# AliBahri94/GM3D

Hardware: AMD Instinct MI355X
Metric: point-clouds/sec pretrain step (N=1024,G=64) (higher is better)
Workload: dtype bf16

## Files before the change

gm3d_amd/csrc/attention.hip:

```cpp
#include "mfma.hpp"

namespace gm3d {

constexpr int HD = 64;
constexpr int VLD = 72;

__device__ __forceinline__ int permk(int s, int j, int hh) { return 16 * s + 8 * (j >> 2) + 4 * hh + (j & 3); }

__device__ __forceinline__ bf16x8 ld8(const bf16_t* p) { return *reinterpret_cast<const bf16x8*>(p); }
__device__ __forceinline__ bf16x8 ld8_perm(const bf16_t* row, int k0, int s, int hh) {
    const bf16x4 a = *reinterpret_cast<const bf16x4*>(row + k0 + 16 * s + 4 * hh);
    const bf16x4 b = *reinterpret_cast<const bf16x4*>(row + k0 + 16 * s + 8 + 4 * hh);
    bf16x8 v;
#pragma unroll
    for (int j = 0; j < 4; ++j) { v[j] = a[j]; v[4 + j] = b[j]; }
    return v;
}
__device__ __forceinline__ bf16x8 ld8_col_perm(const bf16_t* M, int ld, int k0, int s, int hh, int col) {
    bf16x8 v;
#pragma unroll
    for (int j = 0; j < 8; ++j) v[j] = M[(size_t)(k0 + permk(s, j, hh)) * ld + col];
    return v;
}

#define MFMA_F32(a, b, c) __builtin_amdgcn_mfma_f32_32x32x2f32(a, b, c, 0, 0, 0)

__device__ __forceinline__ void stage_bf16(bf16_t* dst , const bf16_t* src, size_t row_stride, int T, int rows) {
    for (int c = threadIdx.x; c < rows * 8; c += blockDim.x) {
        const int row = c >> 3, col = (c & 7) * 8;
        *reinterpret_cast<bf16x8*>(dst + row * VLD + col) = row < T ? ld8(src + (size_t)row * row_stride + col) : zero8();
    }
}
__device__ __forceinline__ int rot(int r, int c) { return r * 64 + ((c + r) & 63); }
__device__ __forceinline__ void stage_f32(float* dst , const float* src, size_t row_stride, int T, int rows) {
    for (int c = threadIdx.x; c < rows * 64; c += blockDim.x) {
        const int row = c >> 6, col = c & 63;
        dst[rot(row, col)] = row < T ? src[(size_t)row * row_stride + col] : 0.f;
    }
}

__device__ __forceinline__ int img_off(int row, int ch) {
    const int f = swz(row);
    return row * 128 + ((ch ^ f) << 4);
}
__device__ __forceinline__ bf16x8 img_row(const unsigned char* img, int row, int ch) {
    return *reinterpret_cast<const bf16x8*>(img + img_off(row, ch));
}
__device__ __forceinline__ bf16x4 img_tr(const unsigned char* img, int row0, int colblk, int lane) {
    const int l16 = lane & 15, q = l16 >> 2, p = l16 & 3;
    const int col = colblk + 4 * p;
    const int addr = img_off(row0 + q, col >> 3) + ((col >> 2) & 1) * 8;
    return __builtin_amdgcn_ds_read_tr16_b64_v4bf16((lds_bf16x4*)(img + addr));
}
__device__ __forceinline__ bf16x8 img_tr8(const unsigned char* img, int k0, int s, int hh, int colblk, int lane) {
    const bf16x4 lo = img_tr(img, k0 + 16 * s + 4 * hh, colblk, lane);
    const bf16x4 hi = img_tr(img, k0 + 16 * s + 8 + 4 * hh, colblk, lane);
    bf16x8 v;
#pragma unroll
    for (int j = 0; j < 4; ++j) { v[j] = lo[j]; v[4 + j] = hi[j]; }
    return v;
}
__device__ __forceinline__ void store_tile_t(unsigned char* img, int row0, const f32x16& x0, const f32x16& x1, int lane, bf16_t* g,
                                             size_t row_stride, int T) {
    const int r = lane & 31, hh = lane >> 5;
#pragma unroll
    for (int dt = 0; dt < 2; ++dt)
#pragma unroll
        for (int g4 = 0; g4 < 4; ++g4) {
            const f32x16& x = dt ? x1 : x0;
            bf16x4 pk;
#pragma unroll
            for (int e = 0; e < 4; ++e) pk[e] = (bf16_t)x[4 * g4 + e];
            *reinterpret_cast<bf16x4*>(img + img_off(row0 + r, 4 * dt + g4) + 8 * hh) = pk;
        }
    __builtin_amdgcn_fence(__ATOMIC_RELEASE, "wavefront");
    __builtin_amdgcn_wave_barrier();
    __builtin_amdgcn_fence(__ATOMIC_ACQUIRE, "wavefront");
#pragma unroll
    for (int i = 0; i < 4; ++i) {
        const int row = (lane >> 3) + 8 * i, ch = lane & 7;
        if (row0 + row < T)
            *reinterpret_cast<uint4*>(g + (size_t)(row0 + row) * row_stride + ch * 8) =
                *reinterpret_cast<const uint4*>(img + img_off(row0 + row, ch));
    }
}

template <int NT>
__device__ __forceinline__ void attn_core_bf16(const unsigned char* Qi, const unsigned char* Ki, const unsigned char* Vi,
                                               unsigned char* Oi, int w, int lane, int T, float scale, bf16_t* outp, size_t os,
                                               float* lsep) {
    const int r = lane & 31, hh = lane >> 5;
    f32x16 st[NT];
#pragma unroll
    for (int t = 0; t < NT; ++t) st[t] = zero16();
    const int qrow = 32 * w + r;
#pragma unroll
    for (int s = 0; s < 4; ++s) {
        const bf16x8 bq = img_row(Qi, qrow, 2 * s + hh);
#pragma unroll
        for (int t = 0; t < NT; ++t) st[t] = mfma_bf16(img_row(Ki, 32 * t + r, 2 * s + hh), bq, st[t]);
    }
    float m = -INFINITY;
#pragma unroll
    for (int t = 0; t < NT; ++t)
#pragma unroll
        for (int g = 0; g < 16; ++g) {
            const int key = 32 * t + crow(g, hh);
            st[t][g] = key < T ? st[t][g] * scale : -INFINITY;
            m = fmaxf(m, st[t][g]);
        }
    m = fmaxf(m, __shfl_xor(m, 32));
    float sum = 0.f;
#pragma unroll
    for (int t = 0; t < NT; ++t)
#pragma unroll
        for (int g = 0; g < 16; ++g) {
            st[t][g] = __expf(st[t][g] - m);
            sum += st[t][g];
        }
    sum += __shfl_xor(sum, 32);
    const float inv = 1.0f / sum;

    f32x16 o0 = zero16(), o1 = zero16();
    const int cb = 16 * ((lane >> 4) & 1);
#pragma unroll
    for (int t = 0; t < NT; ++t)
#pragma unroll
        for (int s = 0; s < 2; ++s) {
            const bf16x8 p = cvt8(st[t], s, inv);
            o0 = mfma_bf16(img_tr8(Vi, 32 * t, s, hh, cb, lane), p, o0);
            o1 = mfma_bf16(img_tr8(Vi, 32 * t, s, hh, 32 + cb, lane), p, o1);
        }
    store_tile_t(Oi, 32 * w, o0, o1, lane, outp, os, T);
    if (lsep && hh == 0 && qrow < T) lsep[qrow] = m + logf(sum);
}

template <int NT>
__global__ __launch_bounds__(64 * NT) void attn_fwd_bf16_kernel(const bf16_t* __restrict__ qkv, bf16_t* __restrict__ out,
                                                                float* __restrict__ lse, int T, int H, float scale) {
    extern __shared__ __attribute__((aligned(16))) unsigned char smem[];
    constexpr int ROWS = 32 * NT, IMG = ROWS * 128;
    unsigned char* Qi = smem;
    unsigned char* Ki = Qi + IMG;
    unsigned char* Vi = Ki + IMG;
    const int b = blockIdx.x / H, h = blockIdx.x % H;
    const int tid = threadIdx.x, lane = tid & 63, w = __builtin_amdgcn_readfirstlane(tid >> 6);
    const int r = lane & 31, hh = lane >> 5;
    const size_t rs = (size_t)3 * H * HD, os = (size_t)H * HD;
    const bf16_t* Qg = qkv + (size_t)b * T * rs + (size_t)h * HD;
    {
        uint4 v[12];
#pragma unroll
        for (int i = 0; i < 12; ++i) {
            const int c = tid + i * 64 * NT;
            const int tile = c / (ROWS * 8), rc = c - tile * (ROWS * 8), row = rc >> 3, ch = rc & 7;
            const int rr = row < T ? row : T - 1;
            v[i] = *reinterpret_cast<const uint4*>(Qg + (size_t)rr * rs + (size_t)tile * os + ch * 8);
        }
#pragma unroll
        for (int i = 0; i < 12; ++i) {
            const int c = tid + i * 64 * NT;
            const int tile = c / (ROWS * 8), rc = c - tile * (ROWS * 8), row = rc >> 3, ch = rc & 7;
            *reinterpret_cast<uint4*>(smem + tile * IMG + img_off(row, ch)) = row < T ? v[i] : make_uint4(0, 0, 0, 0);
        }
    }
    __syncthreads();

    attn_core_bf16<NT>(Qi, Ki, Vi, Qi, w, lane, T, scale, out + (size_t)b * T * os + (size_t)h * HD, os,
                       lse ? lse + ((size_t)b * H + h) * T : nullptr);
}

constexpr int QA_C = 384, QA_KT = QA_C / 64, QA_STAGE = (64 + 192) * 128;

template <int LOOK, bool WRITE_QKV>
__global__ __launch_bounds__(256) void attn_qkv_fwd_bf16_kernel(const bf16_t* __restrict__ hin, const bf16_t* __restrict__ wqkv,
                                                                bf16_t* __restrict__ out, float* __restrict__ lse,
                                                                bf16_t* __restrict__ qkv_out, int T, int H, float scale, int total) {
    extern __shared__ __attribute__((aligned(16))) unsigned char smem[];
    constexpr int NBUF = LOOK + 1;
    const int tid = threadIdx.x, lane = tid & 63, w = __builtin_amdgcn_readfirstlane(tid >> 6);
    const int r = lane & 31, hh = lane >> 5;
    const int logical = xcd_tile(blockIdx.x, gridDim.x);
    if (logical >= total) return;
    const int b = logical / H, h = logical - b * H;
    const unsigned lds0 = lds_addr(smem);

    const int prow = lane >> 3, pslot = lane & 7;
    const bf16_t* src[8];
#pragma unroll
    for (int i = 0; i < 8; ++i) {
        const int p = w + 4 * i;
        if (p < 8) {
            const int row = 8 * p + prow;
            const int t = row < T ? row : T - 1;
            const int f = (((row >> 1) & 1) << 2) | (((row >> 2) & 1) << 1) | ((row >> 3) & 1);
            src[i] = hin + ((size_t)b * T + t) * QA_C + ((pslot ^ f) << 3);
        } else {
            const int row = 8 * (p - 8) + prow;
            const int f = (((row >> 1) & 1) << 2) | (((row >> 2) & 1) << 1) | ((row >> 3) & 1);
            src[i] = wqkv + ((size_t)(row >> 6) * H * HD + (size_t)h * HD + (row & 63)) * QA_C + ((pslot ^ f) << 3);
        }
    }
#define GM3D_QA_STAGE(ST)                                                                        \
    {                                                                                            \
        const unsigned base = lds0 + ((ST) % NBUF) * QA_STAGE;                                   \
        _Pragma("unroll") for (int i = 0; i < 8; ++i) glds16(src[i] + (ST) * 64, base + 1024 * (w + 4 * i)); \
    }
    f32x16 acc[3];
#pragma unroll
    for (int j = 0; j < 3; ++j) acc[j] = zero16();
    const int wm = (w >> 1) * 32, wn = (w & 1) * 96;
#pragma unroll
    for (int s = 0; s < LOOK; ++s) GM3D_QA_STAGE(s)
#define GM3D_QA_ITER(KT_)                                                                                                   \
    {                                                                                                                       \
        asm volatile("s_waitcnt vmcnt(%0) lgkmcnt(0)" ::"n"(8 * ((QA_KT - 1 - (KT_)) < (LOOK - 1) ? (QA_KT - 1 - (KT_)) : (LOOK - 1))) : "memory"); \
        __builtin_amdgcn_s_barrier();                                                                                       \
        if ((KT_) + LOOK < QA_KT) GM3D_QA_STAGE((KT_) + LOOK)                                                               \
        const unsigned char* as = smem + ((KT_) % NBUF) * QA_STAGE;                                                         \
        const unsigned char* ws = as + 64 * 128;                                                                            \
        _Pragma("unroll") for (int s = 0; s < 4; ++s) {                                                                     \
            const bf16x8 fa = img_row(as, wm + r, 2 * s + hh);                                                              \
            _Pragma("unroll") for (int j = 0; j < 3; ++j) acc[j] = mfma_bf16(img_row(ws, wn + 32 * j + r, 2 * s + hh), fa, acc[j]); \
        }                                                                                                                   \
    }
    GM3D_QA_ITER(0) GM3D_QA_ITER(1) GM3D_QA_ITER(2) GM3D_QA_ITER(3) GM3D_QA_ITER(4) GM3D_QA_ITER(5)
#undef GM3D_QA_ITER
#undef GM3D_QA_STAGE
    static_assert((QA_KT - 1) % NBUF != 0, "the last stage must not sit in buffer 0");
    unsigned char* Qi = smem;
    unsigned char* Ki = smem + 8192;
    unsigned char* Vi = smem + 16384;
    unsigned char* Oi = smem + 24576;
    {
        const int token = wm + r;
#pragma unroll
        for (int j = 0; j < 3; ++j) {
            const int col = wn + 32 * j;
            unsigned char* img = smem + (col >> 6) * 8192;
            const int cbase = (col & 63) >> 3;
#pragma unroll
            for (int q = 0; q < 4; ++q) {
                bf16x4 pk;
#pragma unroll
                for (int e = 0; e < 4; ++e) pk[e] = token < T ? (bf16_t)acc[j][4 * q + e] : (bf16_t)0.0f;
                *reinterpret_cast<bf16x4*>(img + img_off(token, cbase + q) + 8 * hh) = pk;
            }
        }
    }
    __syncthreads();
    const size_t os = (size_t)H * HD;
    if (w < 2) {
        attn_core_bf16<2>(Qi, Ki, Vi, Oi, w, lane, T, scale, out + (size_t)b * T * os + (size_t)h * HD, os,
                          lse ? lse + ((size_t)b * H + h) * T : nullptr);
    } else if (WRITE_QKV) {
        bf16_t* g = qkv_out + (size_t)b * T * 3 * os + (size_t)h * HD;
        const int t2 = tid - 128;
#pragma unroll
        for (int i = 0; i < 12; ++i) {
            const int c = t2 + 128 * i;
            const int tile = c >> 9, row = (c >> 3) & 63, ch = c & 7;
            if (row < T)
                *reinterpret_cast<uint4*>(g + (size_t)row * 3 * os + (size_t)tile * os + ch * 8) =
                    *reinterpret_cast<const uint4*>(smem + tile * 8192 + img_off(row, ch));
        }
    }
}

template <int MT>
__global__ __launch_bounds__(64 * MT) void attn_fwd_f32_kernel(const float* __restrict__ qkv, float* __restrict__ out,
                                                               float* __restrict__ lse, int T, int H, float scale) {
    extern __shared__ __attribute__((aligned(16))) float sm[];
    constexpr int ROWS = 32 * MT;
    float* Qs = sm;
    float* Ks = Qs + ROWS * 64;
    float* Vs = Ks + ROWS * 64;
    const int b = blockIdx.x / H, h = blockIdx.x % H;
    const int lane = threadIdx.x & 63, qb = threadIdx.x >> 6;
    const int r = lane & 31, hh = lane >> 5;
    const size_t rs = (size_t)3 * H * HD;
    const float* Qg = qkv + (size_t)b * T * rs + (size_t)h * HD;
    const int NK = (T + 31) >> 5;
    stage_f32(Qs, Qg, rs, T, ROWS);
    stage_f32(Ks, Qg + (size_t)H * HD, rs, T, ROWS);
    stage_f32(Vs, Qg + (size_t)2 * H * HD, rs, T, ROWS);
    __syncthreads();

    f32x16 st[MT];
#pragma unroll
    for (int t = 0; t < MT; ++t) st[t] = zero16();
    const int qrow = 32 * qb + r;
    for (int s = 0; s < 32; ++s) {
        const int d = 2 * s + hh;
        const float bq = Qs[rot(qrow, d)];
#pragma unroll
        for (int t = 0; t < MT; ++t)
            if (t < NK) st[t] = MFMA_F32(Ks[rot(32 * t + r, d)], bq, st[t]);
    }
    float m = -INFINITY;
#pragma unroll
    for (int t = 0; t < MT; ++t)
#pragma unroll
        for (int g = 0; g < 16; ++g) {
            const int key = 32 * t + crow(g, hh);
            st[t][g] = key < T ? st[t][g] * scale : -INFINITY;
            m = fmaxf(m, st[t][g]);
        }
    m = fmaxf(m, __shfl_xor(m, 32));
    float sum = 0.f;
#pragma unroll
    for (int t = 0; t < MT; ++t)
#pragma unroll
        for (int g = 0; g < 16; ++g) {
            st[t][g] = expf(st[t][g] - m);
            sum += st[t][g];
        }
    sum += __shfl_xor(sum, 32);
    const float inv = 1.0f / sum;

    f32x16 o0 = zero16(), o1 = zero16();
#pragma unroll
    for (int s = 0; s < 16; ++s) {
        const int key = crow(s, hh);
#pragma unroll
        for (int t = 0; t < MT; ++t)
            if (t < NK) {
                const float p = st[t][s] * inv;
                o0 = MFMA_F32(p, Vs[rot(32 * t + key, r)], o0);
                o1 = MFMA_F32(p, Vs[rot(32 * t + key, 32 + r)], o1);
            }
    }
    float* og = out + (size_t)b * T * H * HD + (size_t)h * HD;
#pragma unroll
    for (int g = 0; g < 16; ++g) {
        const int q = 32 * qb + crow(g, hh);
        if (q < T) {
            og[(size_t)q * H * HD + r] = o0[g];
            og[(size_t)q * H * HD + 32 + r] = o1[g];
        }
    }
    if (lse && hh == 0 && qrow < T) lse[((size_t)b * H + h) * T + qrow] = m + logf(sum);
}

template <int NT>
__global__ __launch_bounds__(128 * NT) void attn_bwd_bf16_kernel(const bf16_t* __restrict__ qkv, const bf16_t* __restrict__ out,
                                                                const bf16_t* __restrict__ dout, const float* __restrict__ lse,
                                                                bf16_t* __restrict__ dqkv, int T, int H, float scale) {
    extern __shared__ __attribute__((aligned(16))) unsigned char smem[];
    constexpr int ROWS = 32 * NT, IMG = ROWS * 128;
    unsigned char* Qi = smem;
    unsigned char* Ki = Qi + IMG;
    unsigned char* Vi = Ki + IMG;
    unsigned char* Di = Vi + IMG;
    float* Ls = reinterpret_cast<float*>(Di + IMG);
    float* Del = Ls + ROWS;
    const int b = blockIdx.x / H, h = blockIdx.x % H;
    const int tid = threadIdx.x, lane = tid & 63, w = __builtin_amdgcn_readfirstlane(tid >> 6);
    const int r = lane & 31, hh = lane >> 5;
    const size_t rs = (size_t)3 * H * HD, os = (size_t)H * HD;
    const bf16_t* Qg = qkv + (size_t)b * T * rs + (size_t)h * HD;
    const bf16_t* Og = out + (size_t)b * T * os + (size_t)h * HD;
    const bf16_t* Dg = dout + (size_t)b * T * os + (size_t)h * HD;
    {
        uint4 v[6], d[2], o[2];
#pragma unroll
        for (int i = 0; i < 6; ++i) {
            const int c = tid + i * 128 * NT;
            const int tile = c / (ROWS * 8), rc = c - tile * (ROWS * 8), row = rc >> 3, ch = rc & 7;
            const int rr = row < T ? row : T - 1;
            v[i] = *reinterpret_cast<const uint4*>(Qg + (size_t)rr * rs + (size_t)tile * os + ch * 8);
        }
#pragma unroll
        for (int i = 0; i < 2; ++i) {
            const int c = tid + i * 128 * NT, row = c >> 3, ch = c & 7;
            const int rr = row < T ? row : T - 1;
            d[i] = *reinterpret_cast<const uint4*>(Dg + (size_t)rr * os + ch * 8);
            o[i] = *reinterpret_cast<const uint4*>(Og + (size_t)rr * os + ch * 8);
        }
#pragma unroll
        for (int i = 0; i < 6; ++i) {
            const int c = tid + i * 128 * NT;
            const int tile = c / (ROWS * 8), rc = c - tile * (ROWS * 8), row = rc >> 3, ch = rc & 7;
            *reinterpret_cast<uint4*>(smem + tile * IMG + img_off(row, ch)) = row < T ? v[i] : make_uint4(0, 0, 0, 0);
        }
#pragma unroll
        for (int i = 0; i < 2; ++i) {
            const int c = tid + i * 128 * NT, row = c >> 3, ch = c & 7;
            const uint4 dz = row < T ? d[i] : make_uint4(0, 0, 0, 0);
            *reinterpret_cast<uint4*>(Di + img_off(row, ch)) = dz;
            const bf16x8 d8 = *reinterpret_cast<const bf16x8*>(&dz), o8 = *reinterpret_cast<const bf16x8*>(&o[i]);
            float acc = 0.f;
#pragma unroll
            for (int j = 0; j < 8; ++j) acc += (float)o8[j] * (float)d8[j];
            acc += __shfl_xor(acc, 1);
            acc += __shfl_xor(acc, 2);
            acc += __shfl_xor(acc, 4);
            if (ch == 0) {
                Del[row] = acc;
                Ls[row] = row < T ? lse[((size_t)b * H + h) * T + row] : 0.f;
            }
        }
    }
    __syncthreads();

    bf16_t* dQg = dqkv + (size_t)b * T * rs + (size_t)h * HD;
    const int cb = 16 * ((lane >> 4) & 1);
    f32x16 x0 = zero16(), x1 = zero16(), y0 = zero16(), y1 = zero16();
    if (w < NT) {
        const int kt = w;
        const int key = 32 * kt + r;
        for (int qt = 0; qt < NT; ++qt) {
            f32x16 s = zero16(), dp = zero16();
#pragma unroll
            for (int ks = 0; ks < 4; ++ks) {
                const int ch = 2 * ks + hh;
                s = mfma_bf16(img_row(Qi, 32 * qt + r, ch), img_row(Ki, key, ch), s);
                dp = mfma_bf16(img_row(Di, 32 * qt + r, ch), img_row(Vi, key, ch), dp);
            }
#pragma unroll
            for (int g = 0; g < 16; ++g) {
                const int q = 32 * qt + crow(g, hh);
                const float p = (q < T && key < T) ? __expf(s[g] * scale - Ls[q]) : 0.f;
                s[g] = p;
                dp[g] = p * (dp[g] - Del[q]);
            }
#pragma unroll
            for (int ks = 0; ks < 2; ++ks) {
                const bf16x8 pa = cvt8(s, ks, 1.0f);
                const bf16x8 da = cvt8(dp, ks, scale);
                x0 = mfma_bf16(img_tr8(Di, 32 * qt, ks, hh, cb, lane), pa, x0);
                x1 = mfma_bf16(img_tr8(Di, 32 * qt, ks, hh, 32 + cb, lane), pa, x1);
                y0 = mfma_bf16(img_tr8(Qi, 32 * qt, ks, hh, cb, lane), da, y0);
                y1 = mfma_bf16(img_tr8(Qi, 32 * qt, ks, hh, 32 + cb, lane), da, y1);
            }
        }
    }
    else {
        const int qt = w - NT;
        const int q = 32 * qt + r;
        const float lq = Ls[q], dq_ = Del[q];
        for (int kt = 0; kt < NT; ++kt) {
            f32x16 s = zero16(), dp = zero16();
#pragma unroll
            for (int ks = 0; ks < 4; ++ks) {
                const int ch = 2 * ks + hh;
                s = mfma_bf16(img_row(Ki, 32 * kt + r, ch), img_row(Qi, q, ch), s);
                dp = mfma_bf16(img_row(Vi, 32 * kt + r, ch), img_row(Di, q, ch), dp);
            }
#pragma unroll
            for (int g = 0; g < 16; ++g) {
                const int key = 32 * kt + crow(g, hh);
                const float p = (q < T && key < T) ? __expf(s[g] * scale - lq) : 0.f;
                dp[g] = p * (dp[g] - dq_);
            }
#pragma unroll
            for (int ks = 0; ks < 2; ++ks) {
                const bf16x8 da = cvt8(dp, ks, scale);
                x0 = mfma_bf16(img_tr8(Ki, 32 * kt, ks, hh, cb, lane), da, x0);
                x1 = mfma_bf16(img_tr8(Ki, 32 * kt, ks, hh, 32 + cb, lane), da, x1);
            }
        }
    }
    __syncthreads();
    if (w < NT) {
        store_tile_t(Vi, 32 * w, x0, x1, lane, dQg + 2 * os, rs, T);
        store_tile_t(Ki, 32 * w, y0, y1, lane, dQg + os, rs, T);
    } else {
        store_tile_t(Qi, 32 * (w - NT), x0, x1, lane, dQg, rs, T);
    }
}

template <int MT>
__global__ __launch_bounds__(128 * MT) void attn_bwd_f32_kernel(const float* __restrict__ qkv, const float* __restrict__ out,
                                                               const float* __restrict__ dout, const float* __restrict__ lse,
                                                               float* __restrict__ dqkv, int T, int H, float scale) {
    extern __shared__ __attribute__((aligned(16))) float sm[];
    constexpr int ROWS = 32 * MT;
    float* Qs = sm;
    float* Ks = Qs + ROWS * 64;
    float* Vs = Ks + ROWS * 64;
    float* Ds = Vs + ROWS * 64;
    float* Ls = Ds + ROWS * 64;
    float* Del = Ls + ROWS;
    const int b = blockIdx.x / H, h = blockIdx.x % H;
    const int tid = threadIdx.x, lane = tid & 63, w = tid >> 6;
    const int r = lane & 31, hh = lane >> 5;
    const size_t rs = (size_t)3 * H * HD, os = (size_t)H * HD;
    const float* Qg = qkv + (size_t)b * T * rs + (size_t)h * HD;
    const float* Og = out + (size_t)b * T * os + (size_t)h * HD;
    const float* Dg = dout + (size_t)b * T * os + (size_t)h * HD;
    const int NT = (T + 31) >> 5;

    stage_f32(Qs, Qg, rs, T, ROWS);
    stage_f32(Ks, Qg + os, rs, T, ROWS);
    stage_f32(Vs, Qg + 2 * os, rs, T, ROWS);
    stage_f32(Ds, Dg, os, T, ROWS);
    {
        const int q = tid >> 1, half = tid & 1;
        float acc = 0.f;
        if (q < T)
            for (int c = 0; c < 32; ++c) acc += Og[(size_t)q * os + half * 32 + c] * Dg[(size_t)q * os + half * 32 + c];
        acc += __shfl_xor(acc, 1);
        if (half == 0 && q < ROWS) {
            Del[q] = acc;
            Ls[q] = q < T ? lse[((size_t)b * H + h) * T + q] : 0.f;
        }
    }
    __syncthreads();

    float* dQg = dqkv + (size_t)b * T * rs + (size_t)h * HD;
    float* dKg = dQg + os;
    float* dVg = dKg + os;

    if (w < NT) {
        const int kt = w;
        const int key = 32 * kt + r;
        f32x16 dv0 = zero16(), dv1 = zero16(), dk0 = zero16(), dk1 = zero16();
        for (int qt = 0; qt < NT; ++qt) {
            f32x16 s = zero16(), dp = zero16();
            for (int ks = 0; ks < 32; ++ks) {
                const int d = 2 * ks + hh;
                s = MFMA_F32(Qs[rot(32 * qt + r, d)], Ks[rot(key, d)], s);
                dp = MFMA_F32(Ds[rot(32 * qt + r, d)], Vs[rot(key, d)], dp);
            }
#pragma unroll
            for (int g = 0; g < 16; ++g) {
                const int q = 32 * qt + crow(g, hh);
                const float p = (q < T && key < T) ? expf(s[g] * scale - Ls[q]) : 0.f;
                s[g] = p;
                dp[g] = p * (dp[g] - Del[q]) * scale;
            }
#pragma unroll
            for (int ks = 0; ks < 16; ++ks) {
                const int q = 32 * qt + crow(ks, hh);
                dv0 = MFMA_F32(s[ks], Ds[rot(q, r)], dv0);
                dv1 = MFMA_F32(s[ks], Ds[rot(q, 32 + r)], dv1);
                dk0 = MFMA_F32(dp[ks], Qs[rot(q, r)], dk0);
                dk1 = MFMA_F32(dp[ks], Qs[rot(q, 32 + r)], dk1);
            }
        }
#pragma unroll
        for (int g = 0; g < 16; ++g) {
            const int kk = 32 * kt + crow(g, hh);
            if (kk < T) {
                dVg[(size_t)kk * rs + r] = dv0[g];
                dVg[(size_t)kk * rs + 32 + r] = dv1[g];
                dKg[(size_t)kk * rs + r] = dk0[g];
                dKg[(size_t)kk * rs + 32 + r] = dk1[g];
            }
        }
    }
    else {
        const int qt = w - NT;
        const int q = 32 * qt + r;
        const float lq = Ls[q], dq_ = Del[q];
        f32x16 dq0 = zero16(), dq1 = zero16();
        for (int kt = 0; kt < NT; ++kt) {
            f32x16 s = zero16(), dp = zero16();
            for (int ks = 0; ks < 32; ++ks) {
                const int d = 2 * ks + hh;
                s = MFMA_F32(Ks[rot(32 * kt + r, d)], Qs[rot(q, d)], s);
                dp = MFMA_F32(Vs[rot(32 * kt + r, d)], Ds[rot(q, d)], dp);
            }
#pragma unroll
            for (int g = 0; g < 16; ++g) {
                const int key = 32 * kt + crow(g, hh);
                const float p = (q < T && key < T) ? expf(s[g] * scale - lq) : 0.f;
                dp[g] = p * (dp[g] - dq_) * scale;
            }
#pragma unroll
            for (int ks = 0; ks < 16; ++ks) {
                const int key = 32 * kt + crow(ks, hh);
                dq0 = MFMA_F32(dp[ks], Ks[rot(key, r)], dq0);
                dq1 = MFMA_F32(dp[ks], Ks[rot(key, 32 + r)], dq1);
            }
        }
#pragma unroll
        for (int g = 0; g < 16; ++g) {
            const int qq = 32 * qt + crow(g, hh);
            if (qq < T) {
                dQg[(size_t)qq * rs + r] = dq0[g];
                dQg[(size_t)qq * rs + 32 + r] = dq1[g];
            }
        }
    }
}

static int attn_check(const void* a, const void* b, int B, int T, int H, int dtype) {
    if (!a || !b || B < 0 || T < 1 || H < 1) return GM3D_EINVAL;
    if (T > 128) return GM3D_EUNSUPPORTED;
    if (dtype != GM3D_F32 && dtype != GM3D_BF16) return GM3D_EINVAL;
    if ((long long)B * H > 0x7fffffffLL) return GM3D_EUNSUPPORTED;
    return GM3D_OK;
}

}

extern "C" int gm3d_attention_fwd(const void* qkv, void* out, float* lse, int B, int T, int H, float scale,
                                  int dtype, gm3d_stream_t stream) {
    using namespace gm3d;
    int rc = attn_check(qkv, out, B, T, H, dtype);
    if (rc != GM3D_OK) return rc;
    if (B == 0) return GM3D_OK;
    const int nt = (T + 31) / 32;
    if (dtype == GM3D_BF16) {
        const size_t lds = (size_t)3 * 32 * nt * 128;
        return by_int<1, 2, 3, 4>(nt, [&](auto c) {
            constexpr int NT = decltype(c)::value;
            return launch_lds<attn_fwd_bf16_kernel<NT>>(dim3(B * H), dim3(64 * NT), lds, stream, (const bf16_t*)qkv, (bf16_t*)out, lse, T, H,
                                                        scale);
        });
    }
    const int threads = 64 * nt;
    const int rows = T <= 64 ? 64 : 128;
    const size_t lds = sizeof(float) * 3 * rows * 64;
    return by_int<2, 4>(T <= 64 ? 2 : 4, [&](auto c) {
        return launch_lds<attn_fwd_f32_kernel<decltype(c)::value>>(dim3(B * H), dim3(threads), lds, stream, (const float*)qkv, (float*)out,
                                                                   lse, T, H, scale);
    });
}

extern "C" int gm3d_attention_qkv_fwd(const void* h, const void* wqkv, void* out, float* lse, void* qkv_out, int B, int T, int H,
                                      int C, float scale, int dtype, gm3d_stream_t stream) {
    using namespace gm3d;
    if (!h || !wqkv || !out || B < 0 || T < 1 || H < 1) return GM3D_EINVAL;
    if (dtype != GM3D_BF16 || T > 64 || C != QA_C || H * HD != C) return GM3D_EUNSUPPORTED;
    if ((((size_t)h | (size_t)wqkv | (size_t)out | (size_t)qkv_out) & 15)) return GM3D_EUNSUPPORTED;
    if ((long long)B * H > 0x7ffffff0LL) return GM3D_EUNSUPPORTED;
    if (B == 0) return GM3D_OK;
    constexpr int LOOK = 1;
    const size_t lds = (size_t)(LOOK + 1) * QA_STAGE;
    const int total = B * H, grid = (total + 7) / 8 * 8;
    return qkv_out ? launch_lds<attn_qkv_fwd_bf16_kernel<LOOK, true>>(dim3(grid), dim3(256), lds, stream, (const bf16_t*)h, (const bf16_t*)wqkv,
                                 (bf16_t*)out, lse, (bf16_t*)qkv_out, T, H, scale, total)
                   : launch_lds<attn_qkv_fwd_bf16_kernel<LOOK, false>>(dim3(grid), dim3(256), lds, stream, (const bf16_t*)h, (const bf16_t*)wqkv,
                                 (bf16_t*)out, lse, (bf16_t*)nullptr, T, H, scale, total);
}

extern "C" int gm3d_attention_bwd(const void* qkv, const void* out, const void* dout, const float* lse, void* dqkv,
                                  int B, int T, int H, float scale, int dtype, gm3d_stream_t stream) {
    using namespace gm3d;
    int rc = attn_check(qkv, out, B, T, H, dtype);
    if (rc != GM3D_OK) return rc;
    if (!dout || !lse || !dqkv) return GM3D_EINVAL;
    if (B == 0) return GM3D_OK;
    const int nt = (T + 31) / 32;
    if (dtype == GM3D_BF16) {
        const size_t lds = (size_t)4 * 32 * nt * 128 + 2 * 32 * nt * sizeof(float);
        return by_int<1, 2, 3, 4>(nt, [&](auto c) {
            constexpr int NT = decltype(c)::value;
            return launch_lds<attn_bwd_bf16_kernel<NT>>(dim3(B * H), dim3(128 * NT), lds, stream, (const bf16_t*)qkv, (const bf16_t*)out,
                                                        (const bf16_t*)dout, lse, (bf16_t*)dqkv, T, H, scale);
        });
    }
    const int threads = 128 * nt;
    const int rows = T <= 64 ? 64 : 128;
    const size_t lds = sizeof(float) * (4 * rows * 64 + 2 * rows);
    return by_int<2, 4>(T <= 64 ? 2 : 4, [&](auto c) {
        return launch_lds<attn_bwd_f32_kernel<decltype(c)::value>>(dim3(B * H), dim3(threads), lds, stream, (const float*)qkv,
                                                                   (const float*)out, (const float*)dout, lse, (float*)dqkv, T, H, scale);
    });
}
```

gm3d_amd/fused.py:

```python
import weakref

import torch

from ._capi import lib
from . import attention_pad, gemm, wgrads
from . import streams as _streams
from .gemm import bias_gelu_bwd, bias_gelu_fwd
from .ops import _launch, _ptr, _stream, _DT
from .wgrads import async_wgrad, defer_wgrad

LNC = 384


class _WeightCache:

    def __init__(self):
        self._c = {}
        self._pinned = {}
        self._groups = []

    def pin(self, model, dtype=torch.bfloat16, static=False):
        src = [p for p in model.parameters() if p.dim() >= 2 and p.dtype == torch.float32 and p.is_cuda
               and not self._is_pinned(p)]
        if not src:
            return
        dst = [torch.empty_like(p, dtype=dtype) for p in src]
        for p, d in zip(src, dst):
            self._pinned[p.data_ptr()] = (d, weakref.ref(p))
        if static:
            with torch.no_grad():
                torch._foreach_copy_(dst, [p.detach() for p in src])
            return
        self._groups.append(([p.detach() for p in src], dst))
        with torch.no_grad():
            torch._foreach_copy_(dst, self._groups[-1][0])

    def pin_view(self, p, shadow):
        self._pinned[p.data_ptr()] = (shadow, weakref.ref(p))
        gemm.forget_transposes()

    def _is_pinned(self, p):
        hit = self._pinned.get(p.data_ptr())
        return hit is not None and hit[1]() is p

    def refresh(self):
        with torch.no_grad():
            for src, dst in self._groups:
                torch._foreach_copy_(dst, src)

    def get(self, w, dtype):
        if w.dtype == dtype:
            return w
        hit = self._pinned.get(w.data_ptr())
        if hit is not None and hit[1]() is w and hit[0].dtype == dtype:
            return hit[0]
        base = w._base
        if base is not None and base.dtype == w.dtype:
            hit = self._pinned.get(base.data_ptr())
            if hit is not None and hit[1]() is base and hit[0].dtype == dtype and hit[0].numel() == base.numel():
                return torch.as_strided(hit[0], w.size(), w.stride(), hit[0].storage_offset() + w.storage_offset() - base.storage_offset())
        if torch.cuda.is_current_stream_capturing():
            return w.detach().to(dtype)
        key = (w.data_ptr(), dtype, tuple(w.shape))
        hit = self._c.get(key)
        if hit is not None and hit[0] == w._version and hit[2]() is w:
            if w.is_cuda:
                cur = torch.cuda.current_stream(w.device)
                if hit[3] != cur.cuda_stream:
                    cur.wait_event(hit[4])
                    hit[1].record_stream(cur)
            return hit[1]
        with torch.no_grad():
            c = w.detach().to(dtype)
        if len(self._c) > 4096:
            self._c.clear()
        stream_id, done = None, None
        if w.is_cuda:
            cur = torch.cuda.current_stream(w.device)
            stream_id, done = cur.cuda_stream, torch.cuda.Event()
            done.record(cur)
        self._c[key] = (w._version, c, weakref.ref(w), stream_id, done)
        return c


weight_cache = _WeightCache()


def residual_ln_fwd(res, y, bias, rowscale, rows_per_sample, add, gamma, beta, eps, adt, R, want_res=True, h=None):
    dev = gamma.device
    out_res = torch.empty(R, LNC, dtype=torch.float32, device=dev) if want_res else None
    if h is None:
        h = torch.empty(R, LNC, dtype=adt, device=dev)
    mean = torch.empty(R, dtype=torch.float32, device=dev)
    rstd = torch.empty(R, dtype=torch.float32, device=dev)
    _launch("gm3d_residual_ln_fwd", {"R": R, "dtype": str(adt)}, lib.gm3d_residual_ln_fwd, _ptr(res), _ptr(y), _ptr(bias),
            _ptr(rowscale), int(rows_per_sample), _ptr(add), _ptr(gamma), _ptr(beta), float(eps), _ptr(out_res), _ptr(h),
            _ptr(mean), _ptr(rstd), R, LNC, _DT[adt], _stream())
    return out_res, h, mean, rstd


def residual_ln_bwd(dh, gin, x, mean, rstd, gamma, rowscale, rows_per_sample, acc, want_dy, adt, R, dy=None, partial=None,
                    acc_out=None):
    dev = gamma.device
    dx = torch.empty(R, LNC, dtype=torch.float32, device=dev)
    if dy is None and want_dy:
        dy = torch.empty(R, LNC, dtype=adt, device=dev)
    nrows = lib.gm3d_ln_partial_rows(R)
    defer = partial is not None
    if partial is None:
        partial = torch.empty(nrows, 3 * LNC, dtype=torch.float32, device=dev)
    _launch("gm3d_residual_ln_bwd", {"R": R, "dtype": str(adt)}, lib.gm3d_residual_ln_bwd, _ptr(dh), _ptr(gin), _ptr(x),
            _ptr(mean), _ptr(rstd), _ptr(gamma), _ptr(rowscale), int(rows_per_sample), _ptr(dx), _ptr(dy), _ptr(acc),
            _ptr(acc_out), _ptr(partial), R, LNC, _DT[adt], _stream())
    if defer:
        return dx, dy, None
    sums = torch.empty(3, LNC, dtype=torch.float32, device=dev)
    _launch("gm3d_colsum_finish", {"rows": nrows, "cols": 3 * LNC}, lib.gm3d_colsum_finish, _ptr(partial), nrows, 3 * LNC,
            3 * LNC, _ptr(sums), 0, _stream())
    return dx, dy, sums


def finish_batched(partial, out):
    J, rows, cols = partial.shape
    _launch("gm3d_colsum_finish_batched", {"rows": J * rows, "cols": cols}, lib.gm3d_colsum_finish_batched, _ptr(partial), J,
            rows * cols, rows, cols, cols, _ptr(out), cols, _stream())
    return out


def _attention_fwd(qkv, B, T, H, scale, out=None):
    if out is None:
        out = torch.empty(B * T, H * 64, dtype=qkv.dtype, device=qkv.device)
    lse = torch.empty(B, H, T, dtype=torch.float32, device=qkv.device)
    if T > 128:
        return attention_pad.forward(qkv, out, lse, B, T, H, scale)
    _launch("gm3d_attention_fwd", {"B": B, "T": T, "H": H, "dtype": str(qkv.dtype)}, lib.gm3d_attention_fwd, _ptr(qkv),
            _ptr(out), _ptr(lse), B, T, H, float(scale), _DT[qkv.dtype], _stream())
    return out, lse


def _attention_qkv_fwd(h, wqkv, B, T, H, scale, out=None, want_qkv=False, want_lse=False):
    C = h.shape[1]
    if out is None:
        out = torch.empty(B * T, C, dtype=h.dtype, device=h.device)
    lse = torch.empty(B, H, T, dtype=torch.float32, device=h.device) if want_lse else None
    qkv = torch.empty(B * T, 3 * C, dtype=h.dtype, device=h.device) if want_qkv else None
    _launch("gm3d_attention_qkv_fwd", {"B": B, "T": T, "H": H, "C": C, "dtype": str(h.dtype)}, lib.gm3d_attention_qkv_fwd, _ptr(h),
            _ptr(wqkv), _ptr(out), _ptr(lse) if want_lse else None, _ptr(qkv) if want_qkv else None, B, T, H, C, float(scale),
            _DT[h.dtype], _stream())
    return out, lse, qkv


def attention_qkv_supported(h, wqkv, T, H):
    return (h.is_cuda and h.dtype == torch.bfloat16 and wqkv.dtype == torch.bfloat16 and T <= 64 and h.shape[1] == 384 == H * 64
            and h.is_contiguous() and wqkv.is_contiguous() and tuple(wqkv.shape) == (1152, 384)
            and h.data_ptr() % 16 == 0 and wqkv.data_ptr() % 16 == 0)


def _attention_bwd(qkv, out, dout, lse, B, T, H, scale, dqkv=None):
    if dqkv is None:
        dqkv = torch.empty_like(qkv)
    if T > 128:
        return attention_pad.backward(qkv, out, dout, lse, dqkv, B, T, H, scale)
    _launch("gm3d_attention_bwd", {"B": B, "T": T, "H": H, "dtype": str(qkv.dtype)}, lib.gm3d_attention_bwd, _ptr(qkv),
            _ptr(out), _ptr(dout), _ptr(lse), _ptr(dqkv), B, T, H, float(scale), _DT[qkv.dtype], _stream())
    return dqkv


DIRECT_INPUT_GRADS = True
FUSE_QKV_ATTENTION = True
PER_BLOCK = 11


def block_params(block):
    return [block.norm1.weight, block.norm1.bias, block.attn.qkv.weight, block.attn.proj.weight, block.attn.proj.bias,
            block.norm2.weight, block.norm2.bias, block.mlp.fc1.weight, block.mlp.fc1.bias, block.mlp.fc2.weight,
            block.mlp.fc2.bias]


class TransformerStackFn(torch.autograd.Function):

    @staticmethod
    def forward(ctx, x, pos, meta, final_w, final_b, *params):
        with torch.autocast("cuda", enabled=False):
            return TransformerStackFn._forward(ctx, x, pos, meta, final_w, final_b, *params)

    @staticmethod
    def _forward(ctx, x, pos, meta, final_w, final_b, *params):
        g = TransformerStackFn._forward_gen(ctx, x, pos, meta, final_w, final_b, *params)
        while True:
            try:
                next(g)
            except StopIteration as done:
                return done.value

    @staticmethod
    def _forward_gen(ctx, x, pos, meta, final_w, final_b, *params):
        B, T, C = x.shape
        assert C == LNC and len(params) % PER_BLOCK == 0
        nblk = len(params) // PER_BLOCK
        adt, H, scale, eps = meta["adt"], meta["num_heads"], meta["scale"], meta["eps"]
        R = B * T
        posa = pos.reshape(R, C).to(adt).contiguous()
        need = meta["grad"] and any(ctx.needs_input_grad)
        y = bias = rs = None
        if x.dtype == adt and adt != torch.float32:
            res, y = None, x.reshape(R, C).contiguous()
        else:
            res = x.reshape(R, C).float().contiguous()
        saved = []
        dev = x.device
        if need:
            H1 = torch.empty(nblk, R, C, dtype=adt, device=dev)
            A = torch.empty(nblk, R, C, dtype=adt, device=dev)
            H2 = torch.empty(nblk, R, C, dtype=adt, device=dev)
            GG = torch.empty(nblk, R, 4 * C, dtype=adt, device=dev)
        fuse_ln = (gemm.fuse_ln() and adt == torch.bfloat16 and x.is_cuda
                   and all(gemm.supported(posa, weight_cache.get(params[i * PER_BLOCK + k], adt)) or k == 9
                           for i in range(nblk) for k in (2, 3, 7)))
        st1 = None
        for i in range(nblk):
            ln1w, ln1b, wqkv, wproj, bproj, ln2w, ln2b, w1, b1, w2, b2 = params[i * PER_BLOCK:(i + 1) * PER_BLOCK]
            dp1, dp2 = meta["dp"][i]
            if fuse_ln:
                if i == 0:
                    u, h1, m1, r1 = residual_ln_fwd(res, y, bias, rs, T, posa, ln1w, ln1b, eps, adt, R, h=H1[i] if need else None)
                    yield
                    qkv = gemm.mm(h1, weight_cache.get(wqkv, adt))
                else:
                    qkv, m1, r1 = gemm.linear_lna(u16, st1, ln1w, ln1b, eps, weight_cache.get(wqkv, adt), None,
                                                  h_out=H1[i] if need else None, want_stats=need)
                yield
                a, lse = _attention_fwd(qkv, B, T, H, scale, out=A[i] if need else None)
                yield
                x1, x16, st2 = gemm.linear_res(a, weight_cache.get(wproj, adt), bproj, u, dp1, T, None)
                yield
                W1 = weight_cache.get(w1, adt)
                f, g, m2, r2 = gemm.linear_lna(x16, st2, ln2w, ln2b, eps, W1, b1, gelu=True,
                                               f_out=torch.empty(R, W1.shape[0], dtype=adt, device=dev) if need else None,
                                               g_out=GG[i] if need else None, h_out=H2[i] if need else None, want_stats=need)
                yield
                if need:
                    saved += [u, m1, r1, qkv, lse, x1, m2, r2, f]
                if i + 1 < nblk:
                    u, u16, st1 = gemm.linear_res(g, weight_cache.get(w2, adt), b2, x1, dp2, T, posa)
                else:
                    o = gemm.mm(g, weight_cache.get(w2, adt))
                    res, y, bias, rs = x1, o, b2, dp2
                yield
                continue
            u, h1, m1, r1 = residual_ln_fwd(res, y, bias, rs, T, posa, ln1w, ln1b, eps, adt, R, h=H1[i] if need else None)
            yield
            Wq = weight_cache.get(wqkv, adt)
            if FUSE_QKV_ATTENTION and T > 32 and attention_qkv_supported(h1, Wq, T, H):
                a, lse, qkv = _attention_qkv_fwd(h1, Wq, B, T, H, scale, out=A[i] if need else None, want_qkv=need, want_lse=need)
            else:
                qkv = gemm.mm(h1, Wq)
                yield
                a, lse = _attention_fwd(qkv, B, T, H, scale, out=A[i] if need else None)
            yield
            p = gemm.mm(a, weight_cache.get(wproj, adt))
            yield
            x1, h2, m2, r2 = residual_ln_fwd(u, p, bproj, dp1, T, None, ln2w, ln2b, eps, adt, R, h=H2[i] if need else None)
            yield
            W1 = weight_cache.get(w1, adt)
            if gemm.route_gelu(h2, W1)[0] == "split":
                f = gemm.mm(h2, W1)
                yield
                g = bias_gelu_fwd(f, b1, adt, g=GG[i] if need else None)
            else:
                f, g = gemm.mm_gelu(h2, W1, b1, need, g_out=GG[i] if need else None)
            yield
            o = gemm.mm(g, weight_cache.get(w2, adt))
            yield
            if need:
                saved += [u, m1, r1, qkv, lse, x1, m2, r2, f]
            res, y, bias, rs = x1, o, b2, dp2
        xf, hout, mf, rf = residual_ln_fwd(res, y, bias, rs, T, None, final_w, final_b, meta["final_eps"], adt, R,
                                           want_res=need, h=meta.get("hout"))
        if need:
            ctx.save_for_backward(final_w, xf, mf, rf, H1, A, H2, GG, *params, *saved)
        ctx.meta, ctx.shape, ctx.nblk = meta, (B, T, C), nblk
        ctx.in_dtypes = (x.dtype, pos.dtype)
        return hout.view(B, T, C)

    @staticmethod
    def backward(ctx, dout):
        with torch.autocast("cuda", enabled=False):
            return TransformerStackFn._backward(ctx, dout)

    @staticmethod
    def _backward(ctx, dout):
        meta, (B, T, C), nblk = ctx.meta, ctx.shape, ctx.nblk
        adt, H, scale = meta["adt"], meta["num_heads"], meta["scale"]
        R = B * T
        tens = ctx.saved_tensors
        final_w, xf, mf, rf, H1, A, H2, GG = tens[:8]
        params = tens[8:8 + nblk * PER_BLOCK]
        saved = tens[8 + nblk * PER_BLOCK:]
        grads = [None] * (nblk * PER_BLOCK)
        dev = dout.device
        dh = dout.reshape(R, C).to(adt).contiguous()
        DO = torch.empty(nblk, R, C, dtype=adt, device=dev)
        DF = torch.empty(nblk, R, 4 * C, dtype=adt, device=dev)
        DP = torch.empty(nblk, R, C, dtype=adt, device=dev)
        DQ = torch.empty(nblk, R, 3 * C, dtype=adt, device=dev)
        PLN = torch.empty(2 * nblk + 1, lib.gm3d_ln_partial_rows(R), 3 * C, dtype=torch.float32, device=dev)
        SLN = torch.empty(2 * nblk + 1, 3, C, dtype=torch.float32, device=dev)
        w2s = [weight_cache.get(params[i * PER_BLOCK + 9], adt) for i in range(nblk)]
        gelu_bwd = gemm.route_gelu_bwd(dh, w2s[0])
        fuse_mlp_bwd = gelu_bwd[0] != "split"
        if fuse_mlp_bwd:
            W2T, WPT, W1T, WQT = gemm.stacked_transposes(
                [w2s] + [[weight_cache.get(params[i * PER_BLOCK + k], adt) for i in range(nblk)] for k in (3, 7, 2)])
        PGL = torch.empty(nblk, gelu_bwd[2], 4 * C, dtype=torch.float32, device=dev)
        SGL = torch.empty(nblk, 4 * C, dtype=torch.float32, device=dev)
        dp2_last = meta["dp"][nblk - 1][1]
        G, d_o, _ = residual_ln_bwd(dh, None, xf, mf, rf, final_w, dp2_last, T, None, True, adt, R, dy=DO[nblk - 1],
                                    partial=PLN[2 * nblk])
        g_final_w, g_final_b, db2 = SLN[2 * nblk, 0], SLN[2 * nblk, 1], SLN[2 * nblk, 2]
        dpos = torch.zeros(R, C, dtype=torch.float32, device=dev) if nblk == 1 else None
        for i in range(nblk - 1, -1, -1):
            ln1w, ln1b, wqkv, wproj, bproj, ln2w, ln2b, w1, b1, w2, b2 = params[i * PER_BLOCK:(i + 1) * PER_BLOCK]
            u, m1, r1, qkv, lse, x1, m2, r2, f = saved[i * 9:(i + 1) * 9]
            dp1 = meta["dp"][i][0]
            dp2_prev = meta["dp"][i - 1][1] if i > 0 else None
            gi = grads[i * PER_BLOCK:(i + 1) * PER_BLOCK]
            gi[10] = db2
            if fuse_mlp_bwd:
                df = gemm.mm_gelu_bwd(d_o, W2T[i], f, b1, DF[i], PGL[i], gelu_bwd)
            else:
                dg = gemm.mm_nn(d_o, weight_cache.get(w2, adt))
                df, _ = bias_gelu_bwd(dg, f, b1, adt, df=DF[i], partial=PGL[i])
            gi[8] = SGL[i]
            dh2 = gemm.mm(df, W1T[i]) if fuse_mlp_bwd else gemm.mm_nn(df, weight_cache.get(w1, adt))
            dx1, d_p, _ = residual_ln_bwd(dh2, G, x1, m2, r2, ln2w, dp1, T, None, True, adt, R, dy=DP[i],
                                          partial=PLN[2 * i + 1])
            gi[5], gi[6], gi[4] = SLN[2 * i + 1, 0], SLN[2 * i + 1, 1], SLN[2 * i + 1, 2]
            da = gemm.mm(d_p, WPT[i]) if fuse_mlp_bwd else gemm.mm_nn(d_p, weight_cache.get(wproj, adt))
            dqkv = _attention_bwd(qkv, A[i], da, lse, B, T, H, scale, dqkv=DQ[i])
            dh1 = gemm.mm(dqkv, WQT[i]) if fuse_mlp_bwd else gemm.mm_nn(dqkv, weight_cache.get(wqkv, adt))
            last = DIRECT_INPUT_GRADS and i == 0 and nblk > 1 and adt != torch.float32 and ctx.in_dtypes == (adt, adt)
            if last:
                dx_a = torch.empty(R, C, dtype=adt, device=dev)
                dpos_a = torch.empty(R, C, dtype=adt, device=dev)
                G, _, _ = residual_ln_bwd(dh1, dx1, u, m1, r1, ln1w, None, T, dpos, True, adt, R, dy=dx_a, partial=PLN[0],
                                          acc_out=dpos_a)
            else:
                G, d_o, _ = residual_ln_bwd(dh1, dx1, u, m1, r1, ln1w, dp2_prev, T, dpos, i > 0, adt, R,
                                            dy=DO[i - 1] if i > 0 else None, partial=PLN[2 * i])
            if dpos is None:
                dpos = G
            gi[0], gi[1] = SLN[2 * i, 0], SLN[2 * i, 1]
            db2 = SLN[2 * i, 2]
            grads[i * PER_BLOCK:(i + 1) * PER_BLOCK] = gi
        finish_batched(PLN, SLN.view(2 * nblk + 1, 3 * C))
        finish_batched(PGL, SGL)
        grads[9::PER_BLOCK], grads[7::PER_BLOCK], grads[3::PER_BLOCK], grads[2::PER_BLOCK] = wgrads.stack(
            [(DO, GG, params[9::PER_BLOCK]), (DF, H2, params[7::PER_BLOCK]), (DP, A, params[3::PER_BLOCK]), (DQ, H1, params[2::PER_BLOCK])],
            takes_part=True)
        if last:
            return (dx_a.view(B, T, C), dpos_a.view(B, T, C), None, g_final_w, g_final_b) + tuple(grads)
        dx = G.view(B, T, C).to(ctx.in_dtypes[0])
        return (dx, dpos.view(B, T, C).to(ctx.in_dtypes[1]), None, g_final_w, g_final_b) + tuple(grads)


def run_stack(blocks, final_norm, x, pos, training):
    from . import models_mae_learn_loss as M
    blocks = list(blocks)
    adt = torch.bfloat16 if (torch.is_autocast_enabled() and torch.get_autocast_dtype("cuda") == torch.bfloat16) \
        or x.dtype == torch.bfloat16 else torch.float32
    B = x.shape[0]
    probs = []
    for b in blocks:
        p = getattr(b.drop_path, "drop_prob", 0.0)
        probs += [p, p]
    scales = M.drop_path_scales(B, probs, training, x.device)
    dp = [(scales[2 * i], scales[2 * i + 1]) for i in range(len(blocks))]
    meta = {"num_heads": blocks[0].attn.num_heads, "scale": blocks[0].attn.scale, "eps": blocks[0].norm1.eps,
            "final_eps": final_norm.eps, "adt": adt, "dp": dp, "grad": torch.is_grad_enabled()}
    params = []
    for b in blocks:
        params += block_params(b)
    ns = NOGRAD_SPLIT
    if (ns > 1 and x.is_cuda and not training and B % ns == 0 and B // ns >= 16
            and not (torch.is_grad_enabled() and (x.requires_grad or params[0].requires_grad))):
        main = torch.cuda.current_stream()
        h = B // ns
        x, pos = x.contiguous(), pos.contiguous()
        outs = [None] * ns
        streams = [main] + [_split_stream(x.device, j) for j in range(1, ns)]
        for side in streams[1:]:
            _streams.fork(side, main, who="fused.run_stack: parallel inference chain (NOGRAD_SPLIT)")
            x.record_stream(side)
            pos.record_stream(side)
        if LOCKSTEP:
            T_, C_ = x.shape[1], x.shape[2]
            out = torch.empty(B, T_, C_, dtype=adt, device=x.device)
            for side in streams[1:]:
                out.record_stream(side)
            with torch.autocast("cuda", enabled=False), torch.no_grad():
                gens = [TransformerStackFn._forward_gen(_NoCtx(), x[j * h:(j + 1) * h], pos[j * h:(j + 1) * h],
                                                        dict(meta, hout=out[j * h:(j + 1) * h].view(h * T_, C_)), final_norm.weight,
                                                        final_norm.bias, *params) for j in range(ns)]
                live = ns
                while live:
                    for j in range(ns):
                        if gens[j] is None:
                            continue
                        with torch.cuda.stream(streams[j]):
                            try:
                                next(gens[j])
                            except StopIteration as done:
                                outs[j], gens[j] = done.value, None
                                live -= 1
        else:
            for j in range(1, ns):
                with torch.cuda.stream(streams[j]):
                    outs[j] = TransformerStackFn.apply(x[j * h:(j + 1) * h], pos[j * h:(j + 1) * h], meta, final_norm.weight,
                                                       final_norm.bias, *params)
            outs[0] = TransformerStackFn.apply(x[:h], pos[:h], meta, final_norm.weight, final_norm.bias, *params)
        for j in range(1, ns):
            _streams.join(streams[j], main)
            outs[j].record_stream(main)
        return out if LOCKSTEP else torch.cat(outs, dim=0)
    return TransformerStackFn.apply(x, pos, meta, final_norm.weight, final_norm.bias, *params)


class _NoCtx:
    needs_input_grad = ()

    def save_for_backward(self, *a):
        pass


LOCKSTEP = True
NOGRAD_SPLIT = 2
_split_streams = {}


def _split_stream(device, j=1):
    key = (device.type, device.index, j)
    if key not in _split_streams:
        _split_streams[key] = torch.cuda.Stream(device=device)
    return _split_streams[key]
```

Measured before the change: 17000.

## Process two clouds per block in fused QKV-attention kernel, pack short sequences

The fused QKV-projection+attention kernel now stages 128 token rows per block (two clouds, or four clouds of at most 32 tokens in pack mode), so each weight tile loaded from memory feeds twice as many MFMAs. After the projection, every wave pair (or single wave when packed) runs attention for its own cloud, and all waves take part instead of half writing QKV. The fused path is now also taken for T<=32, and a deeper prefetch (LOOK=2) is used when the grid fits within 256 CUs. In exchange the kernel needs more LDS and registers per block and launches fewer blocks, which can lower occupancy.

```diff
diff --git a/gm3d_amd/csrc/attention.hip b/gm3d_amd/csrc/attention.hip
--- a/gm3d_amd/csrc/attention.hip
+++ b/gm3d_amd/csrc/attention.hip
@@ -170,33 +170,37 @@
                        lse ? lse + ((size_t)b * H + h) * T : nullptr);
 }
 
-constexpr int QA_C = 384, QA_KT = QA_C / 64, QA_STAGE = (64 + 192) * 128;
-
-template <int LOOK, bool WRITE_QKV>
+constexpr int QA_C = 384, QA_KT = QA_C / 64, QA_STAGE = (128 + 192) * 128, QA_PIECES = QA_STAGE / 1024 / 4, QA_IMGS = 4 * 8192;
+constexpr int QA_CUS = 256;
+
+template <int LOOK, bool PACK, bool WRITE_QKV>
 __global__ __launch_bounds__(256) void attn_qkv_fwd_bf16_kernel(const bf16_t* __restrict__ hin, const bf16_t* __restrict__ wqkv,
                                                                 bf16_t* __restrict__ out, float* __restrict__ lse,
-                                                                bf16_t* __restrict__ qkv_out, int T, int H, float scale, int total) {
+                                                                bf16_t* __restrict__ qkv_out, int B, int T, int H, float scale,
+                                                                int total) {
     extern __shared__ __attribute__((aligned(16))) unsigned char smem[];
-    constexpr int NBUF = LOOK + 1;
+    constexpr int NBUF = LOOK + 1, CL = PACK ? 4 : 2;
     const int tid = threadIdx.x, lane = tid & 63, w = __builtin_amdgcn_readfirstlane(tid >> 6);
     const int r = lane & 31, hh = lane >> 5;
     const int logical = xcd_tile(blockIdx.x, gridDim.x);
     if (logical >= total) return;
-    const int b = logical / H, h = logical - b * H;
+    const int grp = logical / H, h = logical - grp * H;
     const unsigned lds0 = lds_addr(smem);
 
     const int prow = lane >> 3, pslot = lane & 7;
-    const bf16_t* src[8];
-#pragma unroll
-    for (int i = 0; i < 8; ++i) {
+    const bf16_t* src[QA_PIECES];
+#pragma unroll
+    for (int i = 0; i < QA_PIECES; ++i) {
         const int p = w + 4 * i;
-        if (p < 8) {
+        if (p < 16) {
             const int row = 8 * p + prow;
-            const int t = row < T ? row : T - 1;
+            const int cl = CL * grp + (PACK ? row >> 5 : row >> 6), tok = PACK ? row & 31 : row & 63;
+            const int b = cl < B ? cl : B - 1;
+            const int t = tok < T ? tok : T - 1;
             const int f = (((row >> 1) & 1) << 2) | (((row >> 2) & 1) << 1) | ((row >> 3) & 1);
             src[i] = hin + ((size_t)b * T + t) * QA_C + ((pslot ^ f) << 3);
         } else {
-            const int row = 8 * (p - 8) + prow;
+            const int row = 8 * (p - 16) + prow;
             const int f = (((row >> 1) & 1) << 2) | (((row >> 2) & 1) << 1) | ((row >> 3) & 1);
             src[i] = wqkv + ((size_t)(row >> 6) * H * HD + (size_t)h * HD + (row & 63)) * QA_C + ((pslot ^ f) << 3);
         }
@@ -204,67 +208,80 @@
 #define GM3D_QA_STAGE(ST)                                                                        \
     {                                                                                            \
         const unsigned base = lds0 + ((ST) % NBUF) * QA_STAGE;                                   \
-        _Pragma("unroll") for (int i = 0; i < 8; ++i) glds16(src[i] + (ST) * 64, base + 1024 * (w + 4 * i)); \
-    }
-    f32x16 acc[3];
-#pragma unroll
-    for (int j = 0; j < 3; ++j) acc[j] = zero16();
+        _Pragma("unroll") for (int i = 0; i < QA_PIECES; ++i) glds16(src[i] + (ST) * 64, base + 1024 * (w + 4 * i)); \
+    }
+    f32x16 acc[2][3];
+#pragma unroll
+    for (int c = 0; c < 2; ++c)
+#pragma unroll
+        for (int j = 0; j < 3; ++j) acc[c][j] = zero16();
     const int wm = (w >> 1) * 32, wn = (w & 1) * 96;
 #pragma unroll
     for (int s = 0; s < LOOK; ++s) GM3D_QA_STAGE(s)
 #define GM3D_QA_ITER(KT_)                                                                                                   \
     {                                                                                                                       \
-        asm volatile("s_waitcnt vmcnt(%0) lgkmcnt(0)" ::"n"(8 * ((QA_KT - 1 - (KT_)) < (LOOK - 1) ? (QA_KT - 1 - (KT_)) : (LOOK - 1))) : "memory"); \
+        asm volatile("s_waitcnt vmcnt(%0) lgkmcnt(0)" ::"n"(QA_PIECES * ((QA_KT - 1 - (KT_)) < (LOOK - 1) ? (QA_KT - 1 - (KT_)) : (LOOK - 1))) : "memory"); \
         __builtin_amdgcn_s_barrier();                                                                                       \
         if ((KT_) + LOOK < QA_KT) GM3D_QA_STAGE((KT_) + LOOK)                                                               \
         const unsigned char* as = smem + ((KT_) % NBUF) * QA_STAGE;                                                         \
-        const unsigned char* ws = as + 64 * 128;                                                                            \
+        const unsigned char* ws = as + 128 * 128;                                                                           \
         _Pragma("unroll") for (int s = 0; s < 4; ++s) {                                                                     \
-            const bf16x8 fa = img_row(as, wm + r, 2 * s + hh);                                                              \
-            _Pragma("unroll") for (int j = 0; j < 3; ++j) acc[j] = mfma_bf16(img_row(ws, wn + 32 * j + r, 2 * s + hh), fa, acc[j]); \
+            const bf16x8 fa0 = img_row(as, wm + r, 2 * s + hh);                                                             \
+            const bf16x8 fa1 = img_row(as + 8192, wm + r, 2 * s + hh);                                                      \
+            _Pragma("unroll") for (int j = 0; j < 3; ++j) {                                                                 \
+                const bf16x8 fw = img_row(ws, wn + 32 * j + r, 2 * s + hh);                                                 \
+                acc[0][j] = mfma_bf16(fw, fa0, acc[0][j]);                                                                  \
+                acc[1][j] = mfma_bf16(fw, fa1, acc[1][j]);                                                                  \
+            }                                                                                                               \
         }                                                                                                                   \
     }
     GM3D_QA_ITER(0) GM3D_QA_ITER(1) GM3D_QA_ITER(2) GM3D_QA_ITER(3) GM3D_QA_ITER(4) GM3D_QA_ITER(5)
 #undef GM3D_QA_ITER
 #undef GM3D_QA_STAGE
-    static_assert((QA_KT - 1) % NBUF != 0, "the last stage must not sit in buffer 0");
-    unsigned char* Qi = smem;
-    unsigned char* Ki = smem + 8192;
-    unsigned char* Vi = smem + 16384;
-    unsigned char* Oi = smem + 24576;
-    {
+    static_assert(2 * QA_IMGS <= NBUF * QA_STAGE, "the images must fit the ring");
+    asm volatile("s_waitcnt lgkmcnt(0)" ::: "memory");
+    __builtin_amdgcn_s_barrier();
+#pragma unroll
+    for (int c = 0; c < 2; ++c) {
         const int token = wm + r;
+        const bool live = (PACK ? (token & 31) : token) < T;
 #pragma unroll
         for (int j = 0; j < 3; ++j) {
             const int col = wn + 32 * j;
-            unsigned char* img = smem + (col >> 6) * 8192;
+            unsigned char* img = smem + c * QA_IMGS + (col >> 6) * 8192;
             const int cbase = (col & 63) >> 3;
 #pragma unroll
             for (int q = 0; q < 4; ++q) {
                 bf16x4 pk;
 #pragma unroll
-                for (int e = 0; e < 4; ++e) pk[e] = token < T ? (bf16_t)acc[j][4 * q + e] : (bf16_t)0.0f;
+                for (int e = 0; e < 4; ++e) pk[e] = live ? (bf16_t)acc[c][j][4 * q + e] : (bf16_t)0.0f;
                 *reinterpret_cast<bf16x4*>(img + img_off(token, cbase + q) + 8 * hh) = pk;
             }
         }
     }
     __syncthreads();
+    const int c = w >> 1, w2 = w & 1;
+    const int cl = CL * grp + (PACK ? 2 * c + w2 : c);
+    if (cl >= B) return;
     const size_t os = (size_t)H * HD;
-    if (w < 2) {
-        attn_core_bf16<2>(Qi, Ki, Vi, Oi, w, lane, T, scale, out + (size_t)b * T * os + (size_t)h * HD, os,
-                          lse ? lse + ((size_t)b * H + h) * T : nullptr);
-    } else if (WRITE_QKV) {
-        bf16_t* g = qkv_out + (size_t)b * T * 3 * os + (size_t)h * HD;
-        const int t2 = tid - 128;
+    unsigned char* Qi = smem + c * QA_IMGS + (PACK ? 4096 * w2 : 0);
+    if (WRITE_QKV) {
+        constexpr int RC = PACK ? 32 : 64, NTH = PACK ? 64 : 128;
+        bf16_t* g = qkv_out + (size_t)cl * T * 3 * os + (size_t)h * HD;
+        const int t2 = tid & (NTH - 1);
 #pragma unroll
         for (int i = 0; i < 12; ++i) {
-            const int c = t2 + 128 * i;
-            const int tile = c >> 9, row = (c >> 3) & 63, ch = c & 7;
+            const int cc = t2 + NTH * i;
+            const int tile = cc / (RC * 8), row = (cc >> 3) & (RC - 1), ch = cc & 7;
             if (row < T)
                 *reinterpret_cast<uint4*>(g + (size_t)row * 3 * os + (size_t)tile * os + ch * 8) =
-                    *reinterpret_cast<const uint4*>(smem + tile * 8192 + img_off(row, ch));
-        }
-    }
+                    *reinterpret_cast<const uint4*>(Qi + tile * 8192 + img_off(row, ch));
+        }
+    }
+    bf16_t* outp = out + (size_t)cl * T * os + (size_t)h * HD;
+    float* lsep = lse ? lse + ((size_t)cl * H + h) * T : nullptr;
+    if (PACK) attn_core_bf16<1>(Qi, Qi + 8192, Qi + 16384, Qi + 24576, 0, lane, T, scale, outp, os, lsep);
+    else attn_core_bf16<2>(Qi, Qi + 8192, Qi + 16384, Qi + 24576, w2, lane, T, scale, outp, os, lsep);
 }
 
 template <int MT>
@@ -628,13 +645,17 @@
     if ((((size_t)h | (size_t)wqkv | (size_t)out | (size_t)qkv_out) & 15)) return GM3D_EUNSUPPORTED;
     if ((long long)B * H > 0x7ffffff0LL) return GM3D_EUNSUPPORTED;
     if (B == 0) return GM3D_OK;
-    constexpr int LOOK = 1;
-    const size_t lds = (size_t)(LOOK + 1) * QA_STAGE;
-    const int total = B * H, grid = (total + 7) / 8 * 8;
-    return qkv_out ? launch_lds<attn_qkv_fwd_bf16_kernel<LOOK, true>>(dim3(grid), dim3(256), lds, stream, (const bf16_t*)h, (const bf16_t*)wqkv,
-                                 (bf16_t*)out, lse, (bf16_t*)qkv_out, T, H, scale, total)
-                   : launch_lds<attn_qkv_fwd_bf16_kernel<LOOK, false>>(dim3(grid), dim3(256), lds, stream, (const bf16_t*)h, (const bf16_t*)wqkv,
-                                 (bf16_t*)out, lse, (bf16_t*)nullptr, T, H, scale, total);
+    const bool pack = T <= 32;
+    const int cl = pack ? 4 : 2;
+    const int total = (B + cl - 1) / cl * H, grid = (total + 7) / 8 * 8;
+    const bool deep = total <= QA_CUS;
+    return by_int<0, 1, 2, 3, 4, 5, 6, 7>(4 * (int)deep + 2 * (int)pack + (qkv_out ? 1 : 0), [&](auto c) {
+        constexpr int V = decltype(c)::value, LOOK = V & 4 ? 2 : 1;
+        constexpr bool PACK = (V & 2) != 0, WRITE = (V & 1) != 0;
+        return launch_lds<attn_qkv_fwd_bf16_kernel<LOOK, PACK, WRITE>>(dim3(grid), dim3(256), (size_t)(LOOK + 1) * QA_STAGE, stream,
+                                                                      (const bf16_t*)h, (const bf16_t*)wqkv, (bf16_t*)out, lse,
+                                                                      (bf16_t*)qkv_out, B, T, H, scale, total);
+    });
 }
 
 extern "C" int gm3d_attention_bwd(const void* qkv, const void* out, const void* dout, const float* lse, void* dqkv,
diff --git a/gm3d_amd/fused.py b/gm3d_amd/fused.py
--- a/gm3d_amd/fused.py
+++ b/gm3d_amd/fused.py
@@ -251,7 +251,7 @@
             u, h1, m1, r1 = residual_ln_fwd(res, y, bias, rs, T, posa, ln1w, ln1b, eps, adt, R, h=H1[i] if need else None)
             yield
             Wq = weight_cache.get(wqkv, adt)
-            if FUSE_QKV_ATTENTION and T > 32 and attention_qkv_supported(h1, Wq, T, H):
+            if FUSE_QKV_ATTENTION and attention_qkv_supported(h1, Wq, T, H):
                 a, lse, qkv = _attention_qkv_fwd(h1, Wq, B, T, H, scale, out=A[i] if need else None, want_qkv=need, want_lse=need)
             else:
                 qkv = gemm.mm(h1, Wq)
```

New measurement: 17090 (median of 6 runs). About the same (+0.6%).
